# facebookresearch/nonrigid_nerf

Hardware: NVIDIA H100
Metric: rays/sec (64c+128f samples, 8x256 MLP), example_sequence training step (higher is better)
Workload: dtype f16 (tensor-core operands; f32 accumulate)

## Files before the change

### __graft_entry__.py

```python
import os
import subprocess
import sys

ROOT = os.path.dirname(os.path.abspath(__file__))
if ROOT not in sys.path:
    sys.path.insert(0, ROOT)


def build() -> None:
    subprocess.check_call(["make", "-j", str(min(8, os.cpu_count() or 1)), "-C", os.path.join(ROOT, "nonrigid_nerf_b200", "csrc")])
    subprocess.check_call(["make", "-C", os.path.join(ROOT, "tests", "cuda")])
    import nonrigid_nerf_b200
    from nonrigid_nerf_b200 import _lib

    lib = _lib.load()
    assert lib.nrn_abi_version() == _lib.ABI_VERSION
    import oracle.nrnerf_oracle
    subprocess.check_call([sys.executable, os.path.join(ROOT, "oracle", "make_ref.py")])


def smoke() -> None:
    import numpy as np
    import torch

    import oracle.nrnerf_oracle as O
    from nonrigid_nerf_b200 import _lib, train as T
    from tests import helpers

    dev = "cuda:0"
    seed, n = 4242, 96
    coarse, fine, bender, (cp, fp, bp) = helpers.build_models(O, seed, dev)
    r = O.make_rays(seed, n)
    rnd = O.make_randomness(seed, n, 64, 64)
    lat = r["latents"].clone().to(dev).requires_grad_(True)
    kw = dict(network_query_fn=None, perturb=1.0, N_importance=64, network_fine=fine, N_samples=64, network_fn=coarse,
              ray_bender=bender, use_viewdirs=False, white_bkgd=False, raw_noise_std=1.0, ndc=False, lindisp=False,
              randomness=rnd)
    rgb, disp, acc, extras = T.render(r["rays_o"].to(dev), r["rays_d"].to(dev), chunk=32768, near=r["near"], far=r["far"],
                                      additional_pixel_information={"ray_bending_latents": lat}, detailed_output=True,
                                      retraw=True, **kw)
    tgt = r["target"].to(dev)
    loss = ((rgb - tgt) ** 2).mean() + ((extras["rgb0"] - tgt) ** 2).mean()
    loss.backward()
    _lib.device_error_check()
# ... 17 lines not shown
```

### nonrigid_nerf_b200/csrc/field_bwd.cu

```cuda
#include "field_mma.cuh"

namespace nrn {

namespace {

constexpr int kBwdStageLd = 66;

static_assert(dgrad::step(dgrad::L6T) == dgrad::step(dgrad::L7T) && dgrad::step(dgrad::L5hT) == dgrad::step(dgrad::L7T) &&
              dgrad::step(dgrad::L4T) == dgrad::step(dgrad::L7T) && dgrad::step(dgrad::L3T) == dgrad::step(dgrad::L7T) &&
              dgrad::step(dgrad::L2T) == dgrad::step(dgrad::L7T) && dgrad::step(dgrad::L1T) == dgrad::step(dgrad::L7T),
              "step_at: one default shape; the consumers run L5h^T .. L1^T as one loop");
constexpr uint32_t kSlabA = 2 * dgrad::step(dgrad::L4T).k16 * kChunkBytes;

__device__ __forceinline__ Step step_at(int step) {
  switch (step) {
    case dgrad::HeadT: return step_imm<dgrad::HeadT>();
    case dgrad::L5eT: return step_imm<dgrad::L5eT>();
    case dgrad::L0T: return step_imm<dgrad::L0T>();
    case dgrad::B4T: return step_imm<dgrad::B4T>();
    case dgrad::B3T: return step_imm<dgrad::B3T>();
    case dgrad::B2T: return step_imm<dgrad::B2T>();
    case dgrad::B1T: return step_imm<dgrad::B1T>();
    case dgrad::B0T: return step_imm<dgrad::B0T>();
    default: return step_imm<dgrad::L7T>();
  }
}

__device__ __forceinline__ float clamp_h(float v) { return fminf(fmaxf(v, -65504.f), 65504.f); }

template <int NCOLS, int NR>
__device__ __forceinline__ void epi_mask_store(const float (&acc)[NR], const ReluMask<NCOLS>& m, uint8_t* img, int g) {
  const int r0 = g * kWgRows + acc_r0(), q = acc_q();
#pragma unroll
  for (int j = 0; j < NCOLS / 8; ++j) {
#pragma unroll
    for (int i = 0; i < 2; ++i) {
      const uint32_t g2 = pack_h2_sat(acc[4 * j + 2 * i], acc[4 * j + 2 * i + 1]);
      *reinterpret_cast<uint32_t*>(img + j * kChunkBytes + (r0 + 8 * i) * 16 + 4 * q) = m.apply(i, j, g2);
    }
// ... 1 lines not shown
}

__device__ __forceinline__ float h_lo(uint32_t w) { return __half2float(__ushort_as_half(static_cast<unsigned short>(w & 0xffffu))); }
__device__ __forceinline__ float h_hi(uint32_t w) { return __half2float(__ushort_as_half(static_cast<unsigned short>(w >> 16))); }

__device__ __forceinline__ void pe_backward(const float* de, const uint8_t* __restrict__ e_row, float (&dx)[3]) {
  float e[64];
#pragma unroll
  for (int c = 0; c < 8; ++c) {
    const uint4 w = __ldg(reinterpret_cast<const uint4*>(e_row + c * kChunkBytes));
    e[c * 8 + 0] = h_lo(w.x); e[c * 8 + 1] = h_hi(w.x); e[c * 8 + 2] = h_lo(w.y); e[c * 8 + 3] = h_hi(w.y);
    e[c * 8 + 4] = h_lo(w.z); e[c * 8 + 5] = h_hi(w.z); e[c * 8 + 6] = h_lo(w.w); e[c * 8 + 7] = h_hi(w.w);
  }
#pragma unroll
  for (int d = 0; d < 3; ++d) {
    float acc = de[d];
#pragma unroll
    for (int k = 0; k < 10; ++k) {
      const float f = static_cast<float>(1 << k);
      const float s = e[3 + 6 * k + d], c = e[3 + 6 * k + 3 + d];
      acc += f * (de[3 + 6 * k + d] * c - de[3 + 6 * k + 3 + d] * s);
    }
    dx[d] += acc;
  }
}

}

template <bool HAS_BENDER>
__global__ void __launch_bounds__(kFwdThreads, 1) field_bwd_kernel(const FieldBwdParams p) {
  extern __shared__ __align__(1024) uint8_t smem[];
  uint8_t* act = smem;
  uint8_t* ring_buf = smem + kHBytes;
  float* stage_all = reinterpret_cast<float*>(ring_buf + kRingStages * kRingStageBytes);
  RingShared* sh = reinterpret_cast<RingShared*>(stage_all + 2 * kWgRows * kBwdStageLd);

  const int warp = threadIdx.x >> 5;
  const int lane = threadIdx.x & 31;

  if (threadIdx.x == 0) sh->init();
  __syncthreads();
  const Waiter W{&sh->abort_flag, p.err};
  Ring ring{ring_buf, sh->w_full, sh->w_empty};

  if (warp >= 8) {
    setmaxnreg_dec<kProducerRegs>();
    if (warp == 8 && lane == 0) produce(p.nerf_wT, p.bend_wT, p.n_tiles, 0, HAS_BENDER ? dgrad::kCount : dgrad::B4T, dgrad::B4T, step_at, ring, W);
    return;
  }

  setmaxnreg_inc<kConsumerRegs>();
  const int g = warp >> 2;
  const int tw = threadIdx.x & 127;
  const bool row_thread = tw < kWgRows;
  const int bar = 1 + g;
  const bool wg_leader = tw == 0;
  const int row = g * kWgRows + tw;
  uint8_t* a_row = act + row * 16;
  const uint32_t a_base = smem_u32(act) + g * kWgRows * 16;
  auto a_slab = [&](uint32_t j) { return a_base + j * kSlabA; };
  float* stg = stage_all + g * kWgRows * kBwdStageLd;
  const float* my_stg = stg + tw * kBwdStageLd;

  const float scale = loss_scale(p.amax);
  const float inv_scale = 1.0f / scale;

  for (int tile = blockIdx.x; tile < p.n_tiles; tile += gridDim.x) {
    const long long pt = static_cast<long long>(tile) * kTileM + row;
    const bool valid = row_thread && pt < p.P;
    const uint8_t* st_tile = p.stash + static_cast<long long>(tile) * kStashTileBytes;
    const uint8_t* st = st_tile + row * 16;
    uint8_t* gs = p.gstash + static_cast<long long>(tile) * kGradTileBytes;
    const StashWriter<false> sw{gs, wg_leader, bar, g};
    const uint8_t* mk = p.relu_mask + static_cast<long long>(tile) * kMaskTileBytes;
    auto prefetch_e = [&]() {
      if (wg_leader) tma_prefetch_l2(st_tile + kStE.off, kEBytes);
// ... 110 lines not shown
      epi_mask_store<kMkHb2.cols>(acc, m, act, g);
      sw.ready(kGsYb1, act);
      m.load(mk + kMkHb1.off, g);
      wg_gemm_step<dgrad::B1T>(acc, ring, a_slab, W, 313);
      sw.begin();
      epi_mask_store<kMkHb1.cols>(acc, m, act, g);
      sw.ready(kGsYb0, act);
    }
    {
      Acc<dgrad::B0T> acc;
      wg_gemm_step<dgrad::B0T>(acc, ring, a_slab, W, 314);
      stage_cols<0, 5>(acc, stg, kBwdStageLd);
      wg_bar(bar);
      if (row_thread) {
        float dl[32];
#pragma unroll
        for (int i = 0; i < 32; ++i) dl[i] = my_stg[6 + i] * inv_scale;
        const long long ray = valid ? pt / p.S : -1;
        const long long ray0 = __shfl_sync(0xffffffffu, ray, 0);
        if (__all_sync(0xffffffffu, ray == ray0 && valid)) {
          const float tot = warp_transpose_reduce(dl, lane);
          atomicAdd(p.d_latents + ray0 * kLatent + lane, tot);
        } else if (valid) {
#pragma unroll
          for (int i = 0; i < 32; ++i) atomicAdd(p.d_latents + ray * kLatent + i, dl[i]);
        }
      }
    }
  }
  if (wg_leader) tma_bulk_wait<0>();
}

cudaError_t launch_field_bwd(const FieldBwdParams& p, bool has_bender, int num_sms, cudaStream_t stream) {
  const size_t smem = kHBytes + kRingStages * kRingStageBytes + 2 * kWgRows * kBwdStageLd * sizeof(float) + sizeof(RingShared) + 64;
  return launch_field(has_bender ? field_bwd_kernel<true> : field_bwd_kernel<false>, p, num_sms, smem, stream);
}

}
```

### nonrigid_nerf_b200/csrc/field_fwd.cu

```cuda
#include "field_mma.cuh"

namespace nrn {

namespace {

constexpr int kFwdStageLd = 12;

static_assert(fwd::step(fwd::L2) == fwd::step(fwd::L1) && fwd::step(fwd::L3) == fwd::step(fwd::L1) &&
              fwd::step(fwd::L4) == fwd::step(fwd::L1) && fwd::step(fwd::L6) == fwd::step(fwd::L1) &&
              fwd::step(fwd::L7) == fwd::step(fwd::L1), "step_at: one default shape");
__device__ __forceinline__ Step step_at(int step) {
  switch (step) {
    case fwd::B0: return step_imm<fwd::B0>();
    case fwd::B1: return step_imm<fwd::B1>();
    case fwd::B2: return step_imm<fwd::B2>();
    case fwd::B3: return step_imm<fwd::B3>();
    case fwd::B4: return step_imm<fwd::B4>();
    case fwd::L0: return step_imm<fwd::L0>();
    case fwd::L5: return step_imm<fwd::L5>();
    case fwd::Head: return step_imm<fwd::Head>();
    default: return step_imm<fwd::L1>();
  }
}
__device__ __forceinline__ uint32_t a_operand_offset(int step, uint32_t j) {
  if (step == fwd::B0 || step == fwd::L0) return kHBytes;
  constexpr uint32_t kSlabA = 2 * fwd::step(fwd::L1).k16 * kChunkBytes;
  if (step == fwd::L5) return j == 0 ? kHBytes : (j - 1) * kSlabA;
  if (step < fwd::L0 || step == fwd::Head) return 0;
  return j * kSlabA;
}

template <int NCOLS, bool MASK, int NR>
__device__ __forceinline__ void epi_bias_relu_store(const float (&acc)[NR], const float* __restrict__ bias, uint8_t* img, int g,
                                                    uint8_t* mask_tile, int mask_off) {
  const int r0 = g * kWgRows + acc_r0(), q = acc_q();
  ReluMask<NCOLS> m;
  if constexpr (MASK) m.clear();
#pragma unroll
  for (int j = 0; j < NCOLS / 8; ++j) {
    const float2 b = __ldg(reinterpret_cast<const float2*>(bias + 8 * j + 2 * q));
#pragma unroll
    for (int i = 0; i < 2; ++i) {
      const uint32_t h2 = pack_h2_relu_sat(acc[4 * j + 2 * i] + b.x, acc[4 * j + 2 * i + 1] + b.y);
      *reinterpret_cast<uint32_t*>(img + j * kChunkBytes + (r0 + 8 * i) * 16 + 4 * q) = h2;
      if constexpr (MASK) m.pack(i, j, h2);
    }
  }
  if constexpr (MASK) m.store(mask_tile + mask_off, g);
}

__device__ __forceinline__ void write_pe(const float (&x)[3], uint8_t* dst_row) {
  float f[64];
  f[0] = x[0]; f[1] = x[1]; f[2] = x[2];
  const float kInv2PiHi = 0.15915494f;
  const float kInv2PiLo = 6.4206199e-09f;
#pragma unroll
  for (int d = 0; d < 3; ++d) {
    const float thi = x[d] * kInv2PiHi;
    const float tlo = fmaf(x[d], kInv2PiLo, fmaf(x[d], kInv2PiHi, -thi));
#pragma unroll
    for (int k = 0; k < 10; ++k) {
      const float sc = static_cast<float>(1 << k);
      const float a = thi * sc;
      const float ph = (a - rintf(a)) + tlo * sc;
      const float ang = ph * 6.2831853071795865f;
      f[3 + 6 * k + d] = __sinf(ang);
      f[3 + 6 * k + 3 + d] = __cosf(ang);
    }
  }
  f[63] = 1.f;
#pragma unroll
  for (int c = 0; c < 8; ++c) {
    uint4 pk;
    pk.x = pack_h2(f[c * 8 + 0], f[c * 8 + 1]);
    pk.y = pack_h2(f[c * 8 + 2], f[c * 8 + 3]);
    pk.z = pack_h2(f[c * 8 + 4], f[c * 8 + 5]);
    pk.w = pack_h2(f[c * 8 + 6], f[c * 8 + 7]);
    *reinterpret_cast<uint4*>(dst_row + c * kChunkBytes) = pk;
  }
}

}

template <bool HAS_BENDER, bool TRAIN>
__global__ void __launch_bounds__(kFwdThreads, 1) field_fwd_kernel(const FieldFwdParams p) {
  extern __shared__ __align__(1024) uint8_t smem[];
  uint8_t* act = smem;
  uint8_t* ring_buf = smem + kSlotBytes;
  float* stage_all = reinterpret_cast<float*>(ring_buf + kRingStages * kRingStageBytes);
  RingShared* sh = reinterpret_cast<RingShared*>(stage_all + 2 * kWgRows * kFwdStageLd);

  const int warp = threadIdx.x >> 5;
  const int lane = threadIdx.x & 31;

  if (threadIdx.x == 0) sh->init();
  __syncthreads();
  const Waiter W{&sh->abort_flag, p.err};
  Ring ring{ring_buf, sh->w_full, sh->w_empty};

  if (warp >= 8) {
    setmaxnreg_dec<kProducerRegs>();
    if (warp == 8 && lane == 0) produce(p.bend_w, p.nerf_w, p.n_tiles, HAS_BENDER ? fwd::B0 : fwd::L0, fwd::kCount, fwd::L0, step_at, ring, W);
    return;
  }

  setmaxnreg_inc<kConsumerRegs>();
  const int g = warp >> 2;
  const int tw = threadIdx.x & 127;
  const bool row_thread = tw < kWgRows;
  const int bar = 1 + g;
  const bool wg_leader = tw == 0;
  uint8_t* Hs = act;
  uint8_t* Es = act + kHBytes;
  uint8_t* e_row = Es + (g * kWgRows + tw) * 16;
  const uint32_t a_h = smem_u32(Hs) + g * kWgRows * 16;
  const uint32_t a_e = smem_u32(Es) + g * kWgRows * 16;
  float* stg = stage_all + g * kWgRows * kFwdStageLd;
  float* my_stg = stg + tw * kFwdStageLd;

  for (int tile = blockIdx.x; tile < p.n_tiles; tile += gridDim.x) {
    const long long pt = static_cast<long long>(tile) * kTileM + g * kWgRows + tw;
    const bool valid = row_thread && pt < p.P;
    uint8_t* st = p.stash ? p.stash + static_cast<long long>(tile) * kStashTileBytes : nullptr;
    const StashWriter<true> sw{st, wg_leader, bar, g};
    uint8_t* mk = TRAIN ? p.relu_mask + static_cast<long long>(tile) * kMaskTileBytes : nullptr;
    float x[3] = {0.f, 0.f, 0.f};
    long long ray = 0;
    if (valid) {
      ray = pt / p.S;
      if (p.pts) {
        const float* q = p.pts + pt * p.pts_stride;
        x[0] = __ldg(q + 0); x[1] = __ldg(q + 1); x[2] = __ldg(q + 2);
      } else {
        const float z = __ldg(p.z_vals + pt);
        const float* r = p.rays + ray * 8;
        x[0] = __fadd_rn(__ldg(r + 0), __fmul_rn(__ldg(r + 3), z));
        x[1] = __fadd_rn(__ldg(r + 1), __fmul_rn(__ldg(r + 4), z));
        x[2] = __fadd_rn(__ldg(r + 2), __fmul_rn(__ldg(r + 5), z));
      }
      if (p.d_init) {
        p.d_init[pt * 3 + 0] = x[0]; p.d_init[pt * 3 + 1] = x[1]; p.d_init[pt * 3 + 2] = x[2];
      }
    }
    float rigidity = 0.f;
    if (HAS_BENDER) {
      sw.begin();
// ... 54 lines not shown
        sw.begin();
        epi_bias_relu_store<kMkHb4.cols, TRAIN>(acc, p.bend_bias + fwd::b_off(fwd::B3), Hs, g, mk, kMkHb4.off);
        sw.ready(kStHb4, Hs);
      }
      {
        Acc<fwd::B4> acc;
        wg_gemm_step<fwd::B4>(acc, ring, [&](uint32_t) { return a_h; }, W, 305);
        stage_cols<0, 1>(acc, stg, kFwdStageLd);
        wg_bar(bar);
        if (row_thread) {
          float un[3], ma[3];
#pragma unroll
          for (int d = 0; d < 3; ++d) {
            un[d] = my_stg[d];
            ma[d] = __fmul_rn(rigidity, un[d]);
            if (p.use_scaling) ma[d] = __fmul_rn(ma[d], p.scaling);
          }
          if (valid) {
            if (p.d_unmasked) { p.d_unmasked[pt * 3 + 0] = un[0]; p.d_unmasked[pt * 3 + 1] = un[1]; p.d_unmasked[pt * 3 + 2] = un[2]; }
            if (p.d_masked) { p.d_masked[pt * 3 + 0] = ma[0]; p.d_masked[pt * 3 + 1] = ma[1]; p.d_masked[pt * 3 + 2] = ma[2]; }
            if (p.d_rigid) p.d_rigid[pt] = rigidity;
          }
#pragma unroll
          for (int d = 0; d < 3; ++d) x[d] = __fadd_rn(x[d], ma[d]);
        }
      }
    }
    if (valid && p.d_bent) {
      p.d_bent[pt * 3 + 0] = x[0]; p.d_bent[pt * 3 + 1] = x[1]; p.d_bent[pt * 3 + 2] = x[2];
    }
    sw.begin();
    if (row_thread) write_pe(x, e_row);
    sw.ready(kStE, Es);
#pragma unroll 1
    for (int L = 0; L < 8; ++L) {
      const int step = fwd::L0 + L;
      Acc<fwd::L1> acc;
      const Step s = step_at(step);
      wg_gemm<fwd::step(fwd::L1).N>(acc, ring, s.nslabs, s.k16, [&](uint32_t j) { return a_h + a_operand_offset(step, j); }, W, 310 + L);
      sw.begin();
      epi_bias_relu_store<kMaskHCols, TRAIN>(acc, p.nerf_bias + L * fwd::b_off(fwd::L1), Hs, g, mk, kMkH + L * kMaskHBytes);
      sw.ready(st_h(L + 1), Hs);
    }
    {
      Acc<fwd::Head> acc;
      wg_gemm_step<fwd::Head>(acc, ring, [&](uint32_t) { return a_h; }, W, 320);
      stage_cols<0, 1>(acc, stg, kFwdStageLd);
      wg_bar(bar);
      if (valid) {
        float o[5];
#pragma unroll
        for (int c = 0; c < 5; ++c) o[c] = my_stg[c] + __ldg(p.nerf_bias + fwd::b_off(fwd::Head) + c);
        if (HAS_BENDER && p.use_removal && rigidity >= p.removal) o[3] *= 0.f;
        float* dst = p.raw + pt * p.out_ch;
        for (int c = 0; c < p.out_ch; ++c) dst[c] = o[c];
      }
    }
  }
  if (p.stash && wg_leader) tma_bulk_wait<0>();
}

size_t field_fwd_smem_bytes() {
  return kSlotBytes + kRingStages * kRingStageBytes + 2 * kWgRows * kFwdStageLd * sizeof(float) + sizeof(RingShared) + 64;
}

cudaError_t launch_field_fwd(const FieldFwdParams& p, bool has_bender, int num_sms, cudaStream_t stream) {
  const size_t smem = field_fwd_smem_bytes();
  const bool train = p.relu_mask != nullptr;
  if (has_bender) return launch_field(train ? field_fwd_kernel<true, true> : field_fwd_kernel<true, false>, p, num_sms, smem, stream);
  return launch_field(train ? field_fwd_kernel<false, true> : field_fwd_kernel<false, false>, p, num_sms, smem, stream);
}

}
```

### nonrigid_nerf_b200/csrc/field_mma.cuh

```cuda
#pragma once
#include "nrn_common.cuh"
#include "sm90_ptx.cuh"

namespace nrn {

namespace {

constexpr int kWgRows = kTileM / 2;

struct RingShared {
  uint64_t w_full[kRingStages];
  uint64_t w_empty[kRingStages];
  int abort_flag;
  __device__ __forceinline__ void init() {
    for (int i = 0; i < kRingStages; ++i) {
      mbar_init(&w_full[i], 1);
      mbar_init(&w_empty[i], 8);
    }
    abort_flag = 0;
    fence_mbar_init();
  }
};

struct Ring {
  uint8_t* buf;
  uint64_t* full;
  uint64_t* empty;
  uint32_t stage = 0, phase = 0;
  __device__ __forceinline__ void next() {
    if (++stage == kRingStages) { stage = 0; phase ^= 1u; }
  }
};

__device__ __forceinline__ void ring_put(Ring& r, const uint8_t* src, uint32_t bytes, const Waiter& W) {
  W.wait(&r.empty[r.stage], r.phase ^ 1u, 101);
  uint8_t* dst = r.buf + r.stage * kRingStageBytes;
  mbar_arrive_expect_tx(&r.full[r.stage], bytes);
  for (uint32_t off = 0; off < bytes; off += 16384u) tma_bulk_g2s(dst + off, src + off, min(bytes - off, 16384u), &r.full[r.stage]);
  r.next();
}

template <typename StepAt>
__device__ __forceinline__ void produce(const uint8_t* w_lo, const uint8_t* w_hi, int n_tiles, int first, int last, int split,
                                        StepAt step_at, Ring& ring, const Waiter& W) {
  for (int tile = blockIdx.x; tile < n_tiles; tile += gridDim.x) {
    uint32_t glo = 0, ghi = 0;
#pragma unroll 1
    for (int step = first; step < last; ++step) {
      const Step s = step_at(step);
      const uint8_t* src = step < split ? w_lo + glo : w_hi + ghi;
      for (uint32_t j = 0; j < s.nslabs; ++j) ring_put(ring, src + j * s.slab_bytes, s.slab_bytes, W);
      if (step < split) glo += s.nslabs * s.slab_bytes; else ghi += s.nslabs * s.slab_bytes;
    }
  }
}

template <int N, typename AAddr>
__device__ __forceinline__ void wg_gemm(float (&acc)[N / 2], Ring& r, uint32_t nslabs, uint32_t k16, AAddr a_addr,
                                        const Waiter& W, int code) {
  const int lane = threadIdx.x & 31;
  uint32_t prev = 0;
#pragma unroll
  for (int i = 0; i < N / 2; ++i) acc[i] = 0.f;
#pragma unroll 1
  for (uint32_t j = 0; j < nslabs; ++j) {
    W.wait(&r.full[r.stage], r.phase, code);
    const uint64_t adesc = gmma_desc(a_addr(j), kChunkBytes, 128);
    const uint64_t bdesc = gmma_desc(smem_u32(r.buf + r.stage * kRingStageBytes), N * 16, 128);
    acc_fence(acc);
    wgmma_fence();
#pragma unroll 1
    for (uint32_t k = 0; k < k16; ++k)
      wgmma<N, 0, 0>(acc, gmma_desc_advance(adesc, k * 2 * kChunkBytes), gmma_desc_advance(bdesc, k * 2 * N * 16), (j | k) ? 1u : 0u);
    wgmma_commit();
    if (j > 0) {
      wgmma_wait<1>();
      __syncwarp();
      if (lane == 0) mbar_arrive(&r.empty[prev]);
    }
    prev = r.stage;
    r.next();
  }
  wgmma_wait<0>();
  acc_fence(acc);
  __syncwarp();
  if (lane == 0) mbar_arrive(&r.empty[prev]);
}

template <auto S>
using Acc = float[step(S).N / 2];
template <auto S, typename AAddr>
__device__ __forceinline__ void wg_gemm_step(Acc<S>& acc, Ring& r, AAddr a_addr, const Waiter& W, int code) {
  constexpr Step s = step(S);
  wg_gemm<s.N>(acc, r, s.nslabs, s.k16, a_addr, W, code);
}

template <auto S>
__device__ __forceinline__ Step step_imm() {
  constexpr Step s = step(S);
  return {s.N, s.nslabs, s.slab_bytes, s.k16};
}

__device__ __forceinline__ int acc_r0() { return ((threadIdx.x >> 5) & 3) * 16 + ((threadIdx.x & 31) >> 2); }
__device__ __forceinline__ int acc_q() { return threadIdx.x & 3; }

template <int NCOLS>
struct ReluMask {
  static constexpr int kH = NCOLS > 128 ? 2 : 1;
  uint32_t w[2][kH];
  static __device__ __forceinline__ size_t offset(int g, int i) {
    return static_cast<size_t>(g * kWgRows + acc_r0() + 8 * i) * (16 * kH) + acc_q() * (4 * kH);
  }
  __device__ __forceinline__ void clear() {
#pragma unroll
    for (int i = 0; i < 2; ++i)
#pragma unroll
      for (int h = 0; h < kH; ++h) w[i][h] = 0u;
  }
  __device__ __forceinline__ void pack(int i, int j, uint32_t h2) {
    w[i][j >> 4] |= __hgt2_mask(*reinterpret_cast<const __half2*>(&h2), __float2half2_rn(0.f)) & (0x00010001u << (j & 15));
  }
  __device__ __forceinline__ void store(uint8_t* img, int g) const {
#pragma unroll
    for (int i = 0; i < 2; ++i) {
      if constexpr (kH == 2) *reinterpret_cast<uint2*>(img + offset(g, i)) = make_uint2(w[i][0], w[i][1]);
      else *reinterpret_cast<uint32_t*>(img + offset(g, i)) = w[i][0];
// ... 69 lines not shown
```

### nonrigid_nerf_b200/csrc/nrn_common.cuh

```cuda
#pragma once
#include <cuda_runtime.h>
#include <stdint.h>

namespace nrn {

constexpr int kTileM = 128;
constexpr int kChunkBytes = kTileM * 16;
constexpr int kRingStageBytes = 32768;
constexpr int kRingStages = 4;
constexpr int kFwdThreads = 384;
constexpr int kProducerRegs = 40, kConsumerRegs = 232;
constexpr int kLatent = 32;

struct WImage {
  int rows, chunks;
  __host__ __device__ constexpr int bytes() const { return rows * chunks * 16; }
  __host__ __device__ constexpr WImage t() const { return {8 * chunks, rows / 8}; }
};

namespace fwd {
enum Id : int { B0, B1, B2, B3, B4, L0, L1, L2, L3, L4, L5, L6, L7, Head, kCount };
__host__ __device__ constexpr WImage image(int s) {
  switch (s) {
    case B0: return {96, 6};
    case B1: return {96, 12};
    case B2: return {80, 12};
    case B3: return {64, 8};
    case B4: return {16, 8};
    case L0: return {256, 8};
    case L5: return {256, 40};
    case Head: return {16, 32};
    default: return {256, 32};
  }
}
}

namespace dgrad {
enum Id : int { HeadT, L7T, L6T, L5eT, L5hT, L4T, L3T, L2T, L1T, L0T, B4T, B3T, B2T, B1T, B0T, kCount };
__host__ __device__ constexpr int forward_of(int s) {
  const int f[kCount] = {fwd::Head, fwd::L7, fwd::L6, fwd::L5, fwd::L5, fwd::L4, fwd::L3, fwd::L2, fwd::L1, fwd::L0,
                         fwd::B4, fwd::B3, fwd::B2, fwd::B1, fwd::B0};
  return f[s];
// ... 17 lines not shown
__host__ __device__ constexpr Step step(int s) { return make_step(image(s)); }
__host__ __device__ constexpr int w_off(int s) { int o = 0; for (int i = s < L0 ? B0 : L0; i < s; ++i) o += image(i).bytes(); return o; }
__host__ __device__ constexpr int b_off(int s) { int o = 0; for (int i = s < L0 ? B0 : L0; i < s; ++i) o += image(i).rows; return o; }
}
namespace dgrad {
__host__ __device__ constexpr Step step(int s) { return make_step(image(s)); }
__host__ __device__ constexpr int w_off(int s) { int o = 0; for (int i = s < B4T ? HeadT : B4T; i < s; ++i) o += image(i).bytes(); return o; }
}

constexpr int kNerfWBytes = fwd::w_off(fwd::Head) + fwd::image(fwd::Head).bytes();
constexpr int kNerfBiasFloats = fwd::b_off(fwd::Head) + fwd::image(fwd::Head).rows;
constexpr int kNerfTOffset = kNerfWBytes + kNerfBiasFloats * 4;
constexpr int kNerfTWBytes = dgrad::w_off(dgrad::L0T) + dgrad::image(dgrad::L0T).bytes();
constexpr int kNerfPackedBytes = kNerfTOffset + kNerfTWBytes;
constexpr int kBendWBytes = fwd::w_off(fwd::B4) + fwd::image(fwd::B4).bytes();
constexpr int kBendBiasFloats = fwd::b_off(fwd::B4);
constexpr int kBendTOffset = kBendWBytes + kBendBiasFloats * 4;
constexpr int kBendTWBytes = dgrad::w_off(dgrad::B0T) + dgrad::image(dgrad::B0T).bytes();
constexpr float kBendLoScale = 2048.f;
constexpr int kBendLoOffset = kBendTOffset + kBendTWBytes;
constexpr int kBendTLoOffset = kBendLoOffset + kBendWBytes;
constexpr int kBendPackedBytes = kBendTLoOffset + kBendTWBytes;
static_assert(kNerfWBytes == 991232 && kNerfTWBytes == 991232 && kBendWBytes == 53248 && kBendTWBytes == 53248, "weight images");
static_assert(kNerfBiasFloats == 8 * 256 + 16 && kBendBiasFloats == 96 + 96 + 80 + 64, "biases");

struct Image {
  int off, chunks;
  __host__ __device__ constexpr int end() const { return off + chunks * kChunkBytes; }
  __host__ __device__ constexpr Image next(int c) const { return {end(), c}; }
};
constexpr int kHChunks = fwd::image(fwd::L1).chunks;
constexpr int kHBytes = kHChunks * kChunkBytes;
constexpr int kEBytes = fwd::image(fwd::L0).chunks * kChunkBytes;
constexpr int kSlotBytes = kHBytes + kEBytes;

constexpr Image kStE{0, fwd::image(fwd::L0).chunks};
constexpr int kStH = kStE.end();
__host__ __device__ constexpr Image st_h(int l) { return {kStH + (l - 1) * kHBytes, kHChunks}; }
constexpr Image kStBin{kStH + 8 * kHBytes, fwd::image(fwd::B0).chunks};
constexpr Image kStHb1 = kStBin.next(fwd::image(fwd::B1).chunks);
constexpr Image kStHb2 = kStHb1.next(fwd::image(fwd::B2).chunks);
constexpr Image kStHb3 = kStHb2.next(fwd::image(fwd::B3).chunks);
constexpr Image kStHb4 = kStHb3.next(fwd::image(fwd::B4).chunks);
constexpr int kStashTileBytes = kStHb4.end();
constexpr Image kGsRaw{0, dgrad::image(dgrad::HeadT).chunks};
constexpr int kGsY = kGsRaw.end();
constexpr Image kGsYb4{kGsY + 8 * kHBytes, dgrad::image(dgrad::B4T).chunks};
constexpr Image kGsYb3 = kGsYb4.next(dgrad::image(dgrad::B3T).chunks);
constexpr Image kGsYb2 = kGsYb3.next(dgrad::image(dgrad::B2T).chunks);
constexpr Image kGsYb1 = kGsYb2.next(dgrad::image(dgrad::B1T).chunks);
constexpr Image kGsYb0 = kGsYb1.next(dgrad::image(dgrad::B0T).chunks);
constexpr int kGradTileBytes = kGsYb0.end();
constexpr int kTanTileBytes = kStashTileBytes - kStBin.off;
constexpr int kAdjTileBytes = kGradTileBytes - kGsYb4.off;
__host__ __device__ constexpr Image tan_image(Image st) { return {st.off - kStBin.off, st.chunks}; }
__host__ __device__ constexpr Image adj_image(Image gs) { return {gs.off - kGsYb4.off, gs.chunks}; }

struct MaskImage {
  int off, cols;
  __host__ __device__ constexpr int end() const { return off + kTileM * (cols > 128 ? 32 : 16); }
  __host__ __device__ constexpr MaskImage next(int c) const { return {end(), c}; }
};
constexpr int kMaskHCols = 8 * kHChunks;
constexpr int kMaskHBytes = MaskImage{0, kMaskHCols}.end();
constexpr int kMkH = 0;
constexpr MaskImage kMkHb1 = MaskImage{kMkH + 7 * kMaskHBytes, kMaskHCols}.next(8 * kStHb1.chunks);
constexpr MaskImage kMkHb2 = kMkHb1.next(8 * kStHb2.chunks);
// ... 68 lines not shown
```

### nonrigid_nerf_b200/csrc/sm90_ptx.cuh

```cuda
#pragma once
#include <cuda_runtime.h>
#include <cuda_fp16.h>
#include <cuda_bf16.h>
#include <stdint.h>

namespace nrn {

__device__ __forceinline__ uint32_t smem_u32(const void* p) {
  return static_cast<uint32_t>(__cvta_generic_to_shared(p));
}

__device__ __forceinline__ void mbar_init(uint64_t* bar, uint32_t count) {
  asm volatile("mbarrier.init.shared::cta.b64 [%0], %1;\n" ::"r"(smem_u32(bar)), "r"(count) : "memory");
}
__device__ __forceinline__ void fence_mbar_init() {
  asm volatile("fence.mbarrier_init.release.cluster;\n" ::: "memory");
}
__device__ __forceinline__ void mbar_arrive(uint64_t* bar) {
  asm volatile("mbarrier.arrive.shared::cta.b64 _, [%0];\n" ::"r"(smem_u32(bar)) : "memory");
}
__device__ __forceinline__ void mbar_arrive_expect_tx(uint64_t* bar, uint32_t bytes) {
  asm volatile("mbarrier.arrive.expect_tx.shared::cta.b64 _, [%0], %1;\n" ::"r"(smem_u32(bar)), "r"(bytes)
               : "memory");
}
// ... 148 lines not shown
template <int TA, int TB>
__device__ __forceinline__ void wgmma_m64n96(float (&d)[48], uint64_t adesc, uint64_t bdesc, uint32_t accumulate) {
  asm volatile(
      "{\n\t.reg .pred p;\n\t"
      "setp.ne.b32 p, %50, 0;\n\t"
      "wgmma.mma_async.sync.aligned.m64n96k16.f32.f16.f16 "
      "{%0, %1, %2, %3, %4, %5, %6, %7, %8, %9, %10, %11, %12, %13, %14, %15, %16, %17, %18, %19, %20, %21, %22, %23, %24, %25, %26, %27, %28, %29, %30, %31, %32, %33, %34, %35, %36, %37, %38, %39, %40, %41, %42, %43, %44, %45, %46, %47}, "
      "%48, %49, p, 1, 1, %51, %52;\n\t}\n"
      : "+f"(d[0]), "+f"(d[1]), "+f"(d[2]), "+f"(d[3]), "+f"(d[4]), "+f"(d[5]), "+f"(d[6]), "+f"(d[7]), "+f"(d[8]), "+f"(d[9]), "+f"(d[10]), "+f"(d[11]), "+f"(d[12]), "+f"(d[13]), "+f"(d[14]), "+f"(d[15]), "+f"(d[16]), "+f"(d[17]), "+f"(d[18]), "+f"(d[19]), "+f"(d[20]), "+f"(d[21]), "+f"(d[22]), "+f"(d[23]), "+f"(d[24]), "+f"(d[25]), "+f"(d[26]), "+f"(d[27]), "+f"(d[28]), "+f"(d[29]), "+f"(d[30]), "+f"(d[31]), "+f"(d[32]), "+f"(d[33]), "+f"(d[34]), "+f"(d[35]), "+f"(d[36]), "+f"(d[37]), "+f"(d[38]), "+f"(d[39]), "+f"(d[40]), "+f"(d[41]), "+f"(d[42]), "+f"(d[43]), "+f"(d[44]), "+f"(d[45]), "+f"(d[46]), "+f"(d[47])
      : "l"(adesc), "l"(bdesc), "r"(accumulate), "n"(TA), "n"(TB));
}

template <int TA, int TB>
__device__ __forceinline__ void wgmma_m64n256(float (&d)[128], uint64_t adesc, uint64_t bdesc, uint32_t accumulate) {
  asm volatile(
      "{\n\t.reg .pred p;\n\t"
      "setp.ne.b32 p, %130, 0;\n\t"
      "wgmma.mma_async.sync.aligned.m64n256k16.f32.f16.f16 "
      "{%0, %1, %2, %3, %4, %5, %6, %7, %8, %9, %10, %11, %12, %13, %14, %15, %16, %17, %18, %19, %20, %21, %22, %23, %24, %25, %26, %27, %28, %29, %30, %31, %32, %33, %34, %35, %36, %37, %38, %39, %40, %41, %42, %43, %44, %45, %46, %47, %48, %49, %50, %51, %52, %53, %54, %55, %56, %57, %58, %59, %60, %61, %62, %63, %64, %65, %66, %67, %68, %69, %70, %71, %72, %73, %74, %75, %76, %77, %78, %79, %80, %81, %82, %83, %84, %85, %86, %87, %88, %89, %90, %91, %92, %93, %94, %95, %96, %97, %98, %99, %100, %101, %102, %103, %104, %105, %106, %107, %108, %109, %110, %111, %112, %113, %114, %115, %116, %117, %118, %119, %120, %121, %122, %123, %124, %125, %126, %127}, "
      "%128, %129, p, 1, 1, %131, %132;\n\t}\n"
      : "+f"(d[0]), "+f"(d[1]), "+f"(d[2]), "+f"(d[3]), "+f"(d[4]), "+f"(d[5]), "+f"(d[6]), "+f"(d[7]), "+f"(d[8]), "+f"(d[9]), "+f"(d[10]), "+f"(d[11]), "+f"(d[12]), "+f"(d[13]), "+f"(d[14]), "+f"(d[15]), "+f"(d[16]), "+f"(d[17]), "+f"(d[18]), "+f"(d[19]), "+f"(d[20]), "+f"(d[21]), "+f"(d[22]), "+f"(d[23]), "+f"(d[24]), "+f"(d[25]), "+f"(d[26]), "+f"(d[27]), "+f"(d[28]), "+f"(d[29]), "+f"(d[30]), "+f"(d[31]), "+f"(d[32]), "+f"(d[33]), "+f"(d[34]), "+f"(d[35]), "+f"(d[36]), "+f"(d[37]), "+f"(d[38]), "+f"(d[39]), "+f"(d[40]), "+f"(d[41]), "+f"(d[42]), "+f"(d[43]), "+f"(d[44]), "+f"(d[45]), "+f"(d[46]), "+f"(d[47]), "+f"(d[48]), "+f"(d[49]), "+f"(d[50]), "+f"(d[51]), "+f"(d[52]), "+f"(d[53]), "+f"(d[54]), "+f"(d[55]), "+f"(d[56]), "+f"(d[57]), "+f"(d[58]), "+f"(d[59]), "+f"(d[60]), "+f"(d[61]), "+f"(d[62]), "+f"(d[63]), "+f"(d[64]), "+f"(d[65]), "+f"(d[66]), "+f"(d[67]), "+f"(d[68]), "+f"(d[69]), "+f"(d[70]), "+f"(d[71]), "+f"(d[72]), "+f"(d[73]), "+f"(d[74]), "+f"(d[75]), "+f"(d[76]), "+f"(d[77]), "+f"(d[78]), "+f"(d[79]), "+f"(d[80]), "+f"(d[81]), "+f"(d[82]), "+f"(d[83]), "+f"(d[84]), "+f"(d[85]), "+f"(d[86]), "+f"(d[87]), "+f"(d[88]), "+f"(d[89]), "+f"(d[90]), "+f"(d[91]), "+f"(d[92]), "+f"(d[93]), "+f"(d[94]), "+f"(d[95]), "+f"(d[96]), "+f"(d[97]), "+f"(d[98]), "+f"(d[99]), "+f"(d[100]), "+f"(d[101]), "+f"(d[102]), "+f"(d[103]), "+f"(d[104]), "+f"(d[105]), "+f"(d[106]), "+f"(d[107]), "+f"(d[108]), "+f"(d[109]), "+f"(d[110]), "+f"(d[111]), "+f"(d[112]), "+f"(d[113]), "+f"(d[114]), "+f"(d[115]), "+f"(d[116]), "+f"(d[117]), "+f"(d[118]), "+f"(d[119]), "+f"(d[120]), "+f"(d[121]), "+f"(d[122]), "+f"(d[123]), "+f"(d[124]), "+f"(d[125]), "+f"(d[126]), "+f"(d[127])
      : "l"(adesc), "l"(bdesc), "r"(accumulate), "n"(TA), "n"(TB));
}

template <int N, int TA, int TB>
__device__ __forceinline__ void wgmma(float (&d)[N / 2], uint64_t adesc, uint64_t bdesc, uint32_t accumulate) {
  static_assert(N == 16 || N == 48 || N == 64 || N == 80 || N == 96 || N == 256, "wgmma: N without a wrapper");
  if constexpr (N == 16) wgmma_m64n16<TA, TB>(d, adesc, bdesc, accumulate);
  else if constexpr (N == 48) wgmma_m64n48<TA, TB>(d, adesc, bdesc, accumulate);
  else if constexpr (N == 64) wgmma_m64n64<TA, TB>(d, adesc, bdesc, accumulate);
  else if constexpr (N == 80) wgmma_m64n80<TA, TB>(d, adesc, bdesc, accumulate);
  else if constexpr (N == 96) wgmma_m64n96<TA, TB>(d, adesc, bdesc, accumulate);
  else wgmma_m64n256<TA, TB>(d, adesc, bdesc, accumulate);
}

__device__ __forceinline__ uint32_t pack_h2(float a, float b) {
  __half2 h = __floats2half2_rn(a, b);
  return *reinterpret_cast<uint32_t*>(&h);
}
__device__ __forceinline__ uint32_t pack_h2_relu_sat(float a, float b) {
  uint32_t d;
  asm("cvt.rn.relu.satfinite.f16x2.f32 %0, %1, %2;" : "=r"(d) : "f"(b), "f"(a));
  return d;
}
__device__ __forceinline__ uint32_t pack_h2_sat(float a, float b) {
  uint32_t d;
  asm("cvt.rn.satfinite.f16x2.f32 %0, %1, %2;" : "=r"(d) : "f"(b), "f"(a));
  return d;
}
__device__ __forceinline__ uint32_t pack_bf2(float a, float b) {
  __nv_bfloat162 h = __floats2bfloat162_rn(a, b);
  return *reinterpret_cast<uint32_t*>(&h);
}

constexpr long long kWaitLimitCycles = 1ll << 28;

struct Waiter {
  int* s_abort;
  int* g_err;
  bool paired = false;
  uint32_t partner_abort = 0;
  __device__ __forceinline__ bool wait(uint64_t* bar, uint32_t parity, int code) const {
    if (mbar_try_wait(bar, parity)) return true;
    const long long t0 = clock64();
    while (!mbar_try_wait(bar, parity)) {
      if (*reinterpret_cast<volatile int*>(s_abort)) return false;
// ... 43 lines not shown
```

Measured before the change: 401,300.

## Keep forward hidden activations in registers and feed WGMMA from register A fragments

The forward MLP layers now repack the bias+ReLU epilogue output straight into f16 A-operand register fragments and run the next layer with register-sourced wgmma (m64n256/m64n16 RS variants). This drops the shared-memory round trip of the hidden activations between layers; smem copies are still written only when training needs them for the stash. The skip input at L5 is still read from smem via a leading descriptor GEMM. The freed smem funds a deeper forward weight ring (5 stages vs 4), at the cost of extra register pressure (64 fragment registers alongside the 128-float accumulator) and a possible risk of spills.

Measured after the change: 417,100, median of 6. 3.9% higher.

```diff
diff --git a/__graft_entry__.py b/__graft_entry__.py
--- a/__graft_entry__.py
+++ b/__graft_entry__.py
@@ -10,6 +10,7 @@
 def build() -> None:
     subprocess.check_call(["make", "-j", str(min(8, os.cpu_count() or 1)), "-C", os.path.join(ROOT, "nonrigid_nerf_b200", "csrc")])
     subprocess.check_call(["make", "-C", os.path.join(ROOT, "tests", "cuda")])
+    subprocess.check_call(["make", "-C", os.path.join(ROOT, "tests", "cuda"), "-f", "wgmma_rs_probe.mk"])
     import nonrigid_nerf_b200
     from nonrigid_nerf_b200 import _lib
 
diff --git a/nonrigid_nerf_b200/csrc/field_bwd.cu b/nonrigid_nerf_b200/csrc/field_bwd.cu
--- a/nonrigid_nerf_b200/csrc/field_bwd.cu
+++ b/nonrigid_nerf_b200/csrc/field_bwd.cu
@@ -5,6 +5,10 @@
 namespace {
 
 constexpr int kBwdStageLd = 66;
+constexpr int kBwdRingStages = 4;
+constexpr size_t kBwdSmemBytes = kHBytes + kBwdRingStages * kRingStageBytes + 2 * kWgRows * kBwdStageLd * sizeof(float) +
+                                 sizeof(RingShared<kBwdRingStages>) + 64;
+static_assert(kBwdSmemBytes <= 227 * 1024, "DGRAD kernel: dynamic shared memory per block");
 
 static_assert(dgrad::step(dgrad::L6T) == dgrad::step(dgrad::L7T) && dgrad::step(dgrad::L5hT) == dgrad::step(dgrad::L7T) &&
               dgrad::step(dgrad::L4T) == dgrad::step(dgrad::L7T) && dgrad::step(dgrad::L3T) == dgrad::step(dgrad::L7T) &&
@@ -72,8 +76,8 @@
   extern __shared__ __align__(1024) uint8_t smem[];
   uint8_t* act = smem;
   uint8_t* ring_buf = smem + kHBytes;
-  float* stage_all = reinterpret_cast<float*>(ring_buf + kRingStages * kRingStageBytes);
-  RingShared* sh = reinterpret_cast<RingShared*>(stage_all + 2 * kWgRows * kBwdStageLd);
+  float* stage_all = reinterpret_cast<float*>(ring_buf + kBwdRingStages * kRingStageBytes);
+  auto* sh = reinterpret_cast<RingShared<kBwdRingStages>*>(stage_all + 2 * kWgRows * kBwdStageLd);
 
   const int warp = threadIdx.x >> 5;
   const int lane = threadIdx.x & 31;
@@ -81,7 +85,7 @@
   if (threadIdx.x == 0) sh->init();
   __syncthreads();
   const Waiter W{&sh->abort_flag, p.err};
-  Ring ring{ring_buf, sh->w_full, sh->w_empty};
+  Ring<kBwdRingStages> ring{ring_buf, sh->w_full, sh->w_empty};
 
   if (warp >= 8) {
     setmaxnreg_dec<kProducerRegs>();
@@ -258,8 +262,7 @@
 }
 
 cudaError_t launch_field_bwd(const FieldBwdParams& p, bool has_bender, int num_sms, cudaStream_t stream) {
-  const size_t smem = kHBytes + kRingStages * kRingStageBytes + 2 * kWgRows * kBwdStageLd * sizeof(float) + sizeof(RingShared) + 64;
-  return launch_field(has_bender ? field_bwd_kernel<true> : field_bwd_kernel<false>, p, num_sms, smem, stream);
-}
-
-}
+  return launch_field(has_bender ? field_bwd_kernel<true> : field_bwd_kernel<false>, p, num_sms, kBwdSmemBytes, stream);
+}
+
+}
diff --git a/nonrigid_nerf_b200/csrc/field_fwd.cu b/nonrigid_nerf_b200/csrc/field_fwd.cu
--- a/nonrigid_nerf_b200/csrc/field_fwd.cu
+++ b/nonrigid_nerf_b200/csrc/field_fwd.cu
@@ -5,6 +5,12 @@
 namespace {
 
 constexpr int kFwdStageLd = 12;
+constexpr int kFwdHBytes = kStHb1.chunks * kChunkBytes;
+static_assert(kStHb2.chunks <= kStHb1.chunks && kStHb3.chunks <= kStHb1.chunks && kStHb4.chunks <= kStHb1.chunks, "bender images fit H");
+constexpr int kFwdRingStages = 5;
+constexpr size_t kFwdSmemBytes = kFwdHBytes + kEBytes + kFwdRingStages * kRingStageBytes + 2 * kWgRows * kFwdStageLd * sizeof(float) +
+                                 sizeof(RingShared<kFwdRingStages>) + 64;
+static_assert(kFwdSmemBytes <= 227 * 1024, "forward kernel: dynamic shared memory per block");
 
 static_assert(fwd::step(fwd::L2) == fwd::step(fwd::L1) && fwd::step(fwd::L3) == fwd::step(fwd::L1) &&
               fwd::step(fwd::L4) == fwd::step(fwd::L1) && fwd::step(fwd::L6) == fwd::step(fwd::L1) &&
@@ -22,14 +28,6 @@
     default: return step_imm<fwd::L1>();
   }
 }
-__device__ __forceinline__ uint32_t a_operand_offset(int step, uint32_t j) {
-  if (step == fwd::B0 || step == fwd::L0) return kHBytes;
-  constexpr uint32_t kSlabA = 2 * fwd::step(fwd::L1).k16 * kChunkBytes;
-  if (step == fwd::L5) return j == 0 ? kHBytes : (j - 1) * kSlabA;
-  if (step < fwd::L0 || step == fwd::Head) return 0;
-  return j * kSlabA;
-}
-
 template <int NCOLS, bool MASK, int NR>
 __device__ __forceinline__ void epi_bias_relu_store(const float (&acc)[NR], const float* __restrict__ bias, uint8_t* img, int g,
                                                     uint8_t* mask_tile, int mask_off) {
@@ -47,6 +45,29 @@
     }
   }
   if constexpr (MASK) m.store(mask_tile + mask_off, g);
+}
+
+template <bool TRAIN>
+__device__ __forceinline__ void epi_bias_relu_frag(const float (&acc)[kMaskHCols / 2], const float* __restrict__ bias,
+                                                   uint32_t (&a)[kMaskHCols / 16][4], uint8_t* st_img, int g,
+                                                   uint8_t* mask_tile, int mask_off) {
+  const int r0 = g * kWgRows + acc_r0(), q = acc_q();
+  ReluMask<kMaskHCols> m;
+  if constexpr (TRAIN) m.clear();
+#pragma unroll
+  for (int j = 0; j < kMaskHCols / 8; ++j) {
+    const float2 b = __ldg(reinterpret_cast<const float2*>(bias + 8 * j + 2 * q));
+#pragma unroll
+    for (int i = 0; i < 2; ++i) {
+      const uint32_t h2 = pack_h2_relu_sat(acc[4 * j + 2 * i] + b.x, acc[4 * j + 2 * i + 1] + b.y);
+      frag_pair(a, j, i) = h2;
+      if constexpr (TRAIN) {
+        m.pack(i, j, h2);
+        *reinterpret_cast<uint32_t*>(st_img + j * kChunkBytes + (r0 + 8 * i) * 16 + 4 * q) = h2;
+      }
+    }
+  }
+  if constexpr (TRAIN) m.store(mask_tile + mask_off, g);
 }
 
 __device__ __forceinline__ void write_pe(const float (&x)[3], uint8_t* dst_row) {
@@ -86,9 +107,9 @@
 __global__ void __launch_bounds__(kFwdThreads, 1) field_fwd_kernel(const FieldFwdParams p) {
   extern __shared__ __align__(1024) uint8_t smem[];
   uint8_t* act = smem;
-  uint8_t* ring_buf = smem + kSlotBytes;
-  float* stage_all = reinterpret_cast<float*>(ring_buf + kRingStages * kRingStageBytes);
-  RingShared* sh = reinterpret_cast<RingShared*>(stage_all + 2 * kWgRows * kFwdStageLd);
+  uint8_t* ring_buf = smem + kFwdHBytes + kEBytes;
+  float* stage_all = reinterpret_cast<float*>(ring_buf + kFwdRingStages * kRingStageBytes);
+  auto* sh = reinterpret_cast<RingShared<kFwdRingStages>*>(stage_all + 2 * kWgRows * kFwdStageLd);
 
   const int warp = threadIdx.x >> 5;
   const int lane = threadIdx.x & 31;
@@ -96,7 +117,7 @@
   if (threadIdx.x == 0) sh->init();
   __syncthreads();
   const Waiter W{&sh->abort_flag, p.err};
-  Ring ring{ring_buf, sh->w_full, sh->w_empty};
+  Ring<kFwdRingStages> ring{ring_buf, sh->w_full, sh->w_empty};
 
   if (warp >= 8) {
     setmaxnreg_dec<kProducerRegs>();
@@ -111,7 +132,7 @@
   const int bar = 1 + g;
   const bool wg_leader = tw == 0;
   uint8_t* Hs = act;
-  uint8_t* Es = act + kHBytes;
+  uint8_t* Es = act + kFwdHBytes;
   uint8_t* e_row = Es + (g * kWgRows + tw) * 16;
   const uint32_t a_h = smem_u32(Hs) + g * kWgRows * 16;
   const uint32_t a_e = smem_u32(Es) + g * kWgRows * 16;
@@ -232,19 +253,17 @@
     sw.begin();
     if (row_thread) write_pe(x, e_row);
     sw.ready(kStE, Es);
+    uint32_t h[kMaskHCols / 16][4];
 #pragma unroll 1
     for (int L = 0; L < 8; ++L) {
-      const int step = fwd::L0 + L;
       Acc<fwd::L1> acc;
-      const Step s = step_at(step);
-      wg_gemm<fwd::step(fwd::L1).N>(acc, ring, s.nslabs, s.k16, [&](uint32_t j) { return a_h + a_operand_offset(step, j); }, W, 310 + L);
-      sw.begin();
-      epi_bias_relu_store<kMaskHCols, TRAIN>(acc, p.nerf_bias + L * fwd::b_off(fwd::L1), Hs, g, mk, kMkH + L * kMaskHBytes);
-      sw.ready(st_h(L + 1), Hs);
+      if (L == 0) wg_gemm_step<fwd::L0>(acc, ring, [&](uint32_t) { return a_e; }, W, 310);
+      else wg_gemm_rs<fwd::step(fwd::L1).N, fwd::step(fwd::L1).k16>(acc, h, ring, L == 5, a_e, W, 310 + L);
+      epi_bias_relu_frag<TRAIN>(acc, p.nerf_bias + L * fwd::b_off(fwd::L1), h, st + st_h(L + 1).off, g, mk, kMkH + L * kMaskHBytes);
     }
     {
       Acc<fwd::Head> acc;
-      wg_gemm_step<fwd::Head>(acc, ring, [&](uint32_t) { return a_h; }, W, 320);
+      wg_gemm_rs<fwd::step(fwd::Head).N, fwd::step(fwd::Head).k16>(acc, h, ring, false, 0u, W, 320);
       stage_cols<0, 1>(acc, stg, kFwdStageLd);
       wg_bar(bar);
       if (valid) {
@@ -260,9 +279,7 @@
   if (p.stash && wg_leader) tma_bulk_wait<0>();
 }
 
-size_t field_fwd_smem_bytes() {
-  return kSlotBytes + kRingStages * kRingStageBytes + 2 * kWgRows * kFwdStageLd * sizeof(float) + sizeof(RingShared) + 64;
-}
+size_t field_fwd_smem_bytes() { return kFwdSmemBytes; }
 
 cudaError_t launch_field_fwd(const FieldFwdParams& p, bool has_bender, int num_sms, cudaStream_t stream) {
   const size_t smem = field_fwd_smem_bytes();
diff --git a/nonrigid_nerf_b200/csrc/field_mma.cuh b/nonrigid_nerf_b200/csrc/field_mma.cuh
--- a/nonrigid_nerf_b200/csrc/field_mma.cuh
+++ b/nonrigid_nerf_b200/csrc/field_mma.cuh
@@ -8,12 +8,13 @@
 
 constexpr int kWgRows = kTileM / 2;
 
+template <int S>
 struct RingShared {
-  uint64_t w_full[kRingStages];
-  uint64_t w_empty[kRingStages];
+  uint64_t w_full[S];
+  uint64_t w_empty[S];
   int abort_flag;
   __device__ __forceinline__ void init() {
-    for (int i = 0; i < kRingStages; ++i) {
+    for (int i = 0; i < S; ++i) {
       mbar_init(&w_full[i], 1);
       mbar_init(&w_empty[i], 8);
     }
@@ -22,17 +23,19 @@
   }
 };
 
+template <int S>
 struct Ring {
   uint8_t* buf;
   uint64_t* full;
   uint64_t* empty;
   uint32_t stage = 0, phase = 0;
   __device__ __forceinline__ void next() {
-    if (++stage == kRingStages) { stage = 0; phase ^= 1u; }
-  }
-};
-
-__device__ __forceinline__ void ring_put(Ring& r, const uint8_t* src, uint32_t bytes, const Waiter& W) {
+    if (++stage == S) { stage = 0; phase ^= 1u; }
+  }
+};
+
+template <int S>
+__device__ __forceinline__ void ring_put(Ring<S>& r, const uint8_t* src, uint32_t bytes, const Waiter& W) {
   W.wait(&r.empty[r.stage], r.phase ^ 1u, 101);
   uint8_t* dst = r.buf + r.stage * kRingStageBytes;
   mbar_arrive_expect_tx(&r.full[r.stage], bytes);
@@ -40,9 +43,9 @@
   r.next();
 }
 
-template <typename StepAt>
+template <typename StepAt, int S>
 __device__ __forceinline__ void produce(const uint8_t* w_lo, const uint8_t* w_hi, int n_tiles, int first, int last, int split,
-                                        StepAt step_at, Ring& ring, const Waiter& W) {
+                                        StepAt step_at, Ring<S>& ring, const Waiter& W) {
   for (int tile = blockIdx.x; tile < n_tiles; tile += gridDim.x) {
     uint32_t glo = 0, ghi = 0;
 #pragma unroll 1
@@ -55,8 +58,8 @@
   }
 }
 
-template <int N, typename AAddr>
-__device__ __forceinline__ void wg_gemm(float (&acc)[N / 2], Ring& r, uint32_t nslabs, uint32_t k16, AAddr a_addr,
+template <int N, typename AAddr, int S>
+__device__ __forceinline__ void wg_gemm(float (&acc)[N / 2], Ring<S>& r, uint32_t nslabs, uint32_t k16, AAddr a_addr,
                                         const Waiter& W, int code) {
   const int lane = threadIdx.x & 31;
   uint32_t prev = 0;
@@ -87,11 +90,58 @@
   if (lane == 0) mbar_arrive(&r.empty[prev]);
 }
 
+template <int N, int K16, int KF, int S>
+__device__ __forceinline__ void wg_gemm_rs(float (&acc)[N / 2], uint32_t (&a)[KF][4], Ring<S>& r, bool lead, uint32_t a_lead,
+                                           const Waiter& W, int code) {
+  static_assert(KF % K16 == 0, "whole slabs of A fragments");
+  const int lane = threadIdx.x & 31;
+  uint32_t prev = 0;
+#pragma unroll
+  for (int i = 0; i < N / 2; ++i) acc[i] = 0.f;
+  if (lead) {
+    W.wait(&r.full[r.stage], r.phase, code);
+    const uint64_t adesc = gmma_desc(a_lead, kChunkBytes, 128);
+    const uint64_t bdesc = gmma_desc(smem_u32(r.buf + r.stage * kRingStageBytes), N * 16, 128);
+    acc_fence(acc);
+    wgmma_fence();
+#pragma unroll
+    for (int k = 0; k < K16; ++k)
+      wgmma<N, 0, 0>(acc, gmma_desc_advance(adesc, k * 2 * kChunkBytes), gmma_desc_advance(bdesc, k * 2 * N * 16), k ? 1u : 0u);
+    wgmma_commit();
+    prev = r.stage;
+    r.next();
+  }
+#pragma unroll
+  for (int j = 0; j < KF / K16; ++j) {
+    W.wait(&r.full[r.stage], r.phase, code);
+    const uint64_t bdesc = gmma_desc(smem_u32(r.buf + r.stage * kRingStageBytes), N * 16, 128);
+    acc_fence(acc);
+    frag_fence(a);
+    wgmma_fence();
+#pragma unroll
+    for (int k = 0; k < K16; ++k)
+      wgmma_rs<N, 0>(acc, a[j * K16 + k], gmma_desc_advance(bdesc, k * 2 * N * 16), (lead || j || k) ? 1u : 0u);
+    wgmma_commit();
+    if (lead || j > 0) {
+      wgmma_wait<1>();
+      __syncwarp();
+      if (lane == 0) mbar_arrive(&r.empty[prev]);
+    }
+    prev = r.stage;
+    r.next();
+  }
+  wgmma_wait<0>();
+  acc_fence(acc);
+  frag_fence(a);
+  __syncwarp();
+  if (lane == 0) mbar_arrive(&r.empty[prev]);
+}
+
 template <auto S>
 using Acc = float[step(S).N / 2];
-template <auto S, typename AAddr>
-__device__ __forceinline__ void wg_gemm_step(Acc<S>& acc, Ring& r, AAddr a_addr, const Waiter& W, int code) {
-  constexpr Step s = step(S);
+template <auto ID, typename AAddr, int S>
+__device__ __forceinline__ void wg_gemm_step(Acc<ID>& acc, Ring<S>& r, AAddr a_addr, const Waiter& W, int code) {
+  constexpr Step s = step(ID);
   wg_gemm<s.N>(acc, r, s.nslabs, s.k16, a_addr, W, code);
 }
 
diff --git a/nonrigid_nerf_b200/csrc/nrn_common.cuh b/nonrigid_nerf_b200/csrc/nrn_common.cuh
--- a/nonrigid_nerf_b200/csrc/nrn_common.cuh
+++ b/nonrigid_nerf_b200/csrc/nrn_common.cuh
@@ -7,7 +7,6 @@
 constexpr int kTileM = 128;
 constexpr int kChunkBytes = kTileM * 16;
 constexpr int kRingStageBytes = 32768;
-constexpr int kRingStages = 4;
 constexpr int kFwdThreads = 384;
 constexpr int kProducerRegs = 40, kConsumerRegs = 232;
 constexpr int kLatent = 32;
@@ -91,7 +90,6 @@
 constexpr int kHChunks = fwd::image(fwd::L1).chunks;
 constexpr int kHBytes = kHChunks * kChunkBytes;
 constexpr int kEBytes = fwd::image(fwd::L0).chunks * kChunkBytes;
-constexpr int kSlotBytes = kHBytes + kEBytes;
 
 constexpr Image kStE{0, fwd::image(fwd::L0).chunks};
 constexpr int kStH = kStE.end();
diff --git a/nonrigid_nerf_b200/csrc/sm90_ptx.cuh b/nonrigid_nerf_b200/csrc/sm90_ptx.cuh
--- a/nonrigid_nerf_b200/csrc/sm90_ptx.cuh
+++ b/nonrigid_nerf_b200/csrc/sm90_ptx.cuh
@@ -204,6 +204,46 @@
   else if constexpr (N == 80) wgmma_m64n80<TA, TB>(d, adesc, bdesc, accumulate);
   else if constexpr (N == 96) wgmma_m64n96<TA, TB>(d, adesc, bdesc, accumulate);
   else wgmma_m64n256<TA, TB>(d, adesc, bdesc, accumulate);
+}
+
+template <int TB>
+__device__ __forceinline__ void wgmma_m64n16_rs(float (&d)[8], const uint32_t (&a)[4], uint64_t bdesc, uint32_t accumulate) {
+  asm volatile(
+      "{\n\t.reg .pred p;\n\t"
+      "setp.ne.b32 p, %13, 0;\n\t"
+      "wgmma.mma_async.sync.aligned.m64n16k16.f32.f16.f16 "
+      "{%0, %1, %2, %3, %4, %5, %6, %7}, "
+      "{%8, %9, %10, %11}, %12, p, 1, 1, %14;\n\t}\n"
+      : "+f"(d[0]), "+f"(d[1]), "+f"(d[2]), "+f"(d[3]), "+f"(d[4]), "+f"(d[5]), "+f"(d[6]), "+f"(d[7])
+      : "r"(a[0]), "r"(a[1]), "r"(a[2]), "r"(a[3]), "l"(bdesc), "r"(accumulate), "n"(TB));
+}
+
+template <int TB>
+__device__ __forceinline__ void wgmma_m64n256_rs(float (&d)[128], const uint32_t (&a)[4], uint64_t bdesc, uint32_t accumulate) {
+  asm volatile(
+      "{\n\t.reg .pred p;\n\t"
+      "setp.ne.b32 p, %133, 0;\n\t"
+      "wgmma.mma_async.sync.aligned.m64n256k16.f32.f16.f16 "
+      "{%0, %1, %2, %3, %4, %5, %6, %7, %8, %9, %10, %11, %12, %13, %14, %15, %16, %17, %18, %19, %20, %21, %22, %23, %24, %25, %26, %27, %28, %29, %30, %31, %32, %33, %34, %35, %36, %37, %38, %39, %40, %41, %42, %43, %44, %45, %46, %47, %48, %49, %50, %51, %52, %53, %54, %55, %56, %57, %58, %59, %60, %61, %62, %63, %64, %65, %66, %67, %68, %69, %70, %71, %72, %73, %74, %75, %76, %77, %78, %79, %80, %81, %82, %83, %84, %85, %86, %87, %88, %89, %90, %91, %92, %93, %94, %95, %96, %97, %98, %99, %100, %101, %102, %103, %104, %105, %106, %107, %108, %109, %110, %111, %112, %113, %114, %115, %116, %117, %118, %119, %120, %121, %122, %123, %124, %125, %126, %127}, "
+      "{%128, %129, %130, %131}, %132, p, 1, 1, %134;\n\t}\n"
+      : "+f"(d[0]), "+f"(d[1]), "+f"(d[2]), "+f"(d[3]), "+f"(d[4]), "+f"(d[5]), "+f"(d[6]), "+f"(d[7]), "+f"(d[8]), "+f"(d[9]), "+f"(d[10]), "+f"(d[11]), "+f"(d[12]), "+f"(d[13]), "+f"(d[14]), "+f"(d[15]), "+f"(d[16]), "+f"(d[17]), "+f"(d[18]), "+f"(d[19]), "+f"(d[20]), "+f"(d[21]), "+f"(d[22]), "+f"(d[23]), "+f"(d[24]), "+f"(d[25]), "+f"(d[26]), "+f"(d[27]), "+f"(d[28]), "+f"(d[29]), "+f"(d[30]), "+f"(d[31]), "+f"(d[32]), "+f"(d[33]), "+f"(d[34]), "+f"(d[35]), "+f"(d[36]), "+f"(d[37]), "+f"(d[38]), "+f"(d[39]), "+f"(d[40]), "+f"(d[41]), "+f"(d[42]), "+f"(d[43]), "+f"(d[44]), "+f"(d[45]), "+f"(d[46]), "+f"(d[47]), "+f"(d[48]), "+f"(d[49]), "+f"(d[50]), "+f"(d[51]), "+f"(d[52]), "+f"(d[53]), "+f"(d[54]), "+f"(d[55]), "+f"(d[56]), "+f"(d[57]), "+f"(d[58]), "+f"(d[59]), "+f"(d[60]), "+f"(d[61]), "+f"(d[62]), "+f"(d[63]), "+f"(d[64]), "+f"(d[65]), "+f"(d[66]), "+f"(d[67]), "+f"(d[68]), "+f"(d[69]), "+f"(d[70]), "+f"(d[71]), "+f"(d[72]), "+f"(d[73]), "+f"(d[74]), "+f"(d[75]), "+f"(d[76]), "+f"(d[77]), "+f"(d[78]), "+f"(d[79]), "+f"(d[80]), "+f"(d[81]), "+f"(d[82]), "+f"(d[83]), "+f"(d[84]), "+f"(d[85]), "+f"(d[86]), "+f"(d[87]), "+f"(d[88]), "+f"(d[89]), "+f"(d[90]), "+f"(d[91]), "+f"(d[92]), "+f"(d[93]), "+f"(d[94]), "+f"(d[95]), "+f"(d[96]), "+f"(d[97]), "+f"(d[98]), "+f"(d[99]), "+f"(d[100]), "+f"(d[101]), "+f"(d[102]), "+f"(d[103]), "+f"(d[104]), "+f"(d[105]), "+f"(d[106]), "+f"(d[107]), "+f"(d[108]), "+f"(d[109]), "+f"(d[110]), "+f"(d[111]), "+f"(d[112]), "+f"(d[113]), "+f"(d[114]), "+f"(d[115]), "+f"(d[116]), "+f"(d[117]), "+f"(d[118]), "+f"(d[119]), "+f"(d[120]), "+f"(d[121]), "+f"(d[122]), "+f"(d[123]), "+f"(d[124]), "+f"(d[125]), "+f"(d[126]), "+f"(d[127])
+      : "r"(a[0]), "r"(a[1]), "r"(a[2]), "r"(a[3]), "l"(bdesc), "r"(accumulate), "n"(TB));
+}
+
+template <int N, int TB>
+__device__ __forceinline__ void wgmma_rs(float (&d)[N / 2], const uint32_t (&a)[4], uint64_t bdesc, uint32_t accumulate) {
+  static_assert(N == 16 || N == 256, "wgmma_rs: N without a wrapper");
+  if constexpr (N == 16) wgmma_m64n16_rs<TB>(d, a, bdesc, accumulate);
+  else wgmma_m64n256_rs<TB>(d, a, bdesc, accumulate);
+}
+template <int KF>
+__device__ __forceinline__ uint32_t& frag_pair(uint32_t (&a)[KF][4], int j, int i) { return a[j >> 1][2 * (j & 1) + i]; }
+template <int KF>
+__device__ __forceinline__ void frag_fence(uint32_t (&a)[KF][4]) {
+#pragma unroll
+  for (int k = 0; k < KF; ++k)
+#pragma unroll
+    for (int i = 0; i < 4; ++i) asm volatile("" : "+r"(a[k][i])::"memory");
 }
 
 __device__ __forceinline__ uint32_t pack_h2(float a, float b) {
```
